# barbararoessle/e2e_multi_view_matching

Hardware: AMD Instinct MI355X
Metric: image-pairs/sec @1024 kpts + pose AUC@5/10/20deg vs reference (higher is better)
Workload: dtype f16x2 (fp32 operands carried as 2 fp16 planes hi + 2^-11 lo', 22 significant bits, 3 fp16-MFMA products, fp32 accumulate; same 1e-4 / bit-exact-index parity bar); 1 GPU; configs[1]: tuple_size=2 (1 pair per tuple), 1024 keypoints, 256-dim f32 descriptors, GNN 9x1 = 18 layers, 100 Sinkhorn iters, batch 32 tuples/GPU = 32 pairs/GPU, w8pt pose per pair; pairs_per_gpu=32, global_pairs=32, weights=random init (timed), identity-like for the AUC leg, parallelism=tuple-sharded x1

## Files before the change

### e2e_multi_view_matching_amd/build.py

```python
import hashlib
import os
import subprocess
import sys

HERE = os.path.dirname(os.path.abspath(__file__))
CSRC = os.path.join(HERE, "csrc")
LIB = os.path.join(HERE, "libe2emv.so")
SOURCES = ["ctx.hip", "weights.hip", "gemm.hip", "attention.hip", "gemm3.hip", "gemm_x3.hip", "gemm_h2.hip", "gemm_p2.hip", "gemm_p2c.hip", "attention_p2.hip", "attention_p2w.hip", "p2_tools.hip", "attention3.hip", "split3_api.hip", "sinkhorn.hip", "sinkhorn_stream.hip", "sinkhorn_resident.hip", "sinkhorn_regs.hip", "sinkhorn_regs2.hip", "pose.hip", "ba2view.hip", "gtmatch.hip",
           "mvinit.hip", "mvinit_device.hip", "mvba.hip", "mvba_backward.hip", "mvtracks.hip", "mvransac.hip", "ransac.hip", "superpoint.hip", "forward.hip", "train.hip", "comm.hip"]
REGISTER_WINDOW = ("sinkhorn_regs.hip", ("sinkhorn_resident128", "sinkhorn_resident2k"), 56)
REGISTER_WINDOW_W = ("sinkhorn_regs2.hip", ("sinkhorn_resident128w",), 64)
FLAGS = ["--offload-arch=gfx950", "-O3", "-std=c++17", "-fPIC", "-fvisibility=hidden", "-fvisibility-inlines-hidden", "-ffp-contract=fast", "-Wno-unused-result"]


def _stamp():
    h = hashlib.sha256()
    for f in sorted(f for f in os.listdir(CSRC) if f.endswith((".hip", ".h")) and os.path.isfile(os.path.join(CSRC, f))) + ["../../include/e2emv.h"]:
        with open(os.path.join(CSRC, f), "rb") as fh:
            h.update(fh.read())
    h.update(" ".join(FLAGS).encode())
    return h.hexdigest()


def build_library(force=False, verbose=False):
    hipcc = os.environ.get("HIPCC", "/opt/rocm/bin/hipcc")
    stamp_file = os.path.join(HERE, "csrc", ".build_stamp")
    stamp = _stamp()
    if not force and os.path.exists(LIB) and os.path.exists(stamp_file) and open(stamp_file).read() == stamp:
        return LIB
    _build(hipcc, os.path.join(HERE, "build"), LIB, verbose)
    with open(stamp_file, "w") as fh:
        fh.write(stamp)
    return LIB


def _check_window(asm_file, kernel, window, accumulation):
    import re
    txt = open(asm_file).read()
    n = 0
    for m in re.finditer(r"^(_Z\w*%s\w*):" % kernel, txt, re.M):
        end = txt.index(".end_amdhsa_kernel", m.end())
        dstart = txt.rfind(".amdhsa_kernel " + m.group(1), m.end(), end)
        if dstart < 0:
            raise RuntimeError(f"{m.group(1)}: no .amdhsa_kernel header in front of .end_amdhsa_kernel")
        body, desc = txt[m.end():dstart], txt[dstart:end]
        total = 512 if accumulation else 256
        if not re.search(r"\.amdhsa_next_free_vgpr\s+%d\b" % total, desc) or not re.search(r"\.amdhsa_accum_offset\s+256\b", desc):
            raise RuntimeError(f"{m.group(1)}: the wave is not allocated " + ("256 + 256 registers" if accumulation else "256 vector registers and no accumulation registers"))
        if not accumulation and not re.search(r"\.amdhsa_private_segment_fixed_size\s+0\b", desc):
            raise RuntimeError(f"{m.group(1)}: the kernel uses scratch memory")
        files = "va" if accumulation else "v"
        inasm = False
        for line in body.split("\n"):
            code = line.split(";")[0]
            if not accumulation:
                if re.search(r"\bscratch_\w+", code):
                    raise RuntimeError(f"{m.group(1)}: the kernel uses scratch memory: {line.strip()}")
                if re.search(r"\ba(\d+|\[\d+:\d+\])(?![\w.])", code) or "accvgpr" in code:
                    raise RuntimeError(f"{m.group(1)}: an accumulation register: {line.strip()}")
            if "#ASMSTART" in line:
                inasm = True
            elif "#ASMEND" in line:
                inasm = False
            elif not inasm:
                regs = [int(x) for x in re.findall(r"\b[%s](\d+)\b" % files, code)] + [int(x) for x in re.findall(r"\b[%s]\[\d+:(\d+)\]" % files, code)]
                if regs and max(regs) >= window:
                    raise RuntimeError(f"{m.group(1)}: compiler-generated code touches a register outside its window: {line.strip()}")
        n += 1
    if n == 0:
        raise RuntimeError(f"{kernel}: not found in {asm_file}")
    return n


def check_register_window(asm_file, kernel, window):
    return _check_window(asm_file, kernel, window, True)


def check_register_window_vgpr(asm_file, kernel, window):
    return _check_window(asm_file, kernel, window, False)


def _build(hipcc, objdir, lib, verbose):
    os.makedirs(objdir, exist_ok=True)
    if any("tgsplit" in f for f in FLAGS):
        raise RuntimeError("libe2emv is built for CU mode: -mtgsplit breaks the in-workgroup hand-off of gemm_p2c.hip")
    procs = []
    kept = (REGISTER_WINDOW[0], REGISTER_WINDOW_W[0])
    for src in SOURCES:
        obj = os.path.join(objdir, src.replace(".hip", ".o"))
        cmd = [hipcc] + FLAGS + ["-c", os.path.join(CSRC, src), "-o", obj]
        cwd = None
        if src in kept:
            stem = src.replace(".hip", "")
            cwd = os.path.join(objdir, stem + "_temps")
            os.makedirs(cwd, exist_ok=True)
            cmd.insert(1, "-save-temps=obj")
            cmd[-1] = os.path.join(cwd, stem + ".o")
        procs.append((src, obj, subprocess.Popen(cmd, stdout=subprocess.PIPE, stderr=subprocess.STDOUT, text=True, cwd=cwd)))
    objs = []
    for src, obj, p in procs:
        out, _ = p.communicate()
        if p.returncode != 0:
            raise RuntimeError(f"hipcc failed on {src}:\n{out}")
        if verbose and out.strip():
            print(out)
        objs.append(obj)
    import shutil
    for (src, kernels, window), check in ((REGISTER_WINDOW, check_register_window), (REGISTER_WINDOW_W, check_register_window_vgpr)):
        stem = src.replace(".hip", "")
        temps = os.path.join(objdir, stem + "_temps")
        shutil.copyfile(os.path.join(temps, stem + ".o"), os.path.join(objdir, stem + ".o"))
        asm_file = os.path.join(objdir, stem + ".s")
        shutil.copyfile(os.path.join(temps, stem + "-hip-amdgcn-amd-amdhsa-gfx950.s"), asm_file)
        for kernel in kernels:
            check(asm_file, kernel, window)
    vs = os.path.join(objdir, "e2emv.map")
    with open(vs, "w") as fh:
        fh.write("{ global: e2emv_*; local: *; };\n")
    cmd = [hipcc, "--offload-arch=gfx950", "-shared", "-fPIC", "-o", lib] + objs + ["-Wl,-rpath,/opt/rocm/lib", "-Wl,--version-script=" + vs]
    r = subprocess.run(cmd, stdout=subprocess.PIPE, stderr=subprocess.STDOUT, text=True)
    if r.returncode != 0:
        raise RuntimeError(f"link failed:\n{r.stdout}")
    return lib


if __name__ == "__main__":
    print(build_library(force="--force" in sys.argv, verbose=True))
```

### e2e_multi_view_matching_amd/csrc/attention_p2w.hip

```cpp
#include <algorithm>
#include <type_traits>

#include "attention_p2.h"

namespace e2emv {

typedef __attribute__((ext_vector_type(16))) float aw_f32x16;

constexpr int AW_QT = 256;
constexpr int AW_TILEB = 64 * 256;
constexpr int AW_REGB = 2 * AW_TILEB;
constexpr int AW_PART_F = 68;
constexpr float AW_SINV = 1.f / P2_QS, AW_PLOG = 7.f, AW_LIMIT = 60000.f;

__device__ __forceinline__ void aw_wait_q(p2_f16x8 (&q)[2][2][4]) {
    asm volatile("s_waitcnt vmcnt(16)"
                 : "+a"(q[0][0][0]), "+a"(q[0][0][1]), "+a"(q[0][0][2]), "+a"(q[0][0][3]), "+a"(q[0][1][0]), "+a"(q[0][1][1]), "+a"(q[0][1][2]), "+a"(q[0][1][3]),
                   "+a"(q[1][0][0]), "+a"(q[1][0][1]), "+a"(q[1][0][2]), "+a"(q[1][0][3]), "+a"(q[1][1][0]), "+a"(q[1][1][1]), "+a"(q[1][1][2]), "+a"(q[1][1][3])
                 :: "memory");
}

template <int I, int N, class F>
__device__ __forceinline__ void aw_for(F&& f) {
    if constexpr (I < N) {
        f(std::integral_constant<int, I>{});
        aw_for<I + 1, N>(f);
    }
}

__device__ __forceinline__ unsigned aw_cvt_pk(float v0, float v1) {
    const p2_f32x2 vv = {v0, v1};
    return __builtin_bit_cast(unsigned, __builtin_convertvector(vv, p2_f16x2));
}
__device__ __forceinline__ float aw_fma(float a, float b, float c) {
    float d;
    asm volatile("v_fma_f32 %0, %1, %2, %3" : "=v"(d) : "v"(a), "v"(b), "v"(c));
    return d;
}
__device__ __forceinline__ float aw_exp2(float a) {
    float d;
    asm volatile("v_exp_f32 %0, %1" : "=v"(d) : "v"(a));
    return d;
}
__device__ __forceinline__ void aw_acc(float& sum, float a) { asm volatile("v_add_f32 %0, %0, %1" : "+v"(sum) : "v"(a)); }
__device__ __forceinline__ unsigned aw_cvt_pk_v(float v0, float v1) {
    unsigned d;
    asm volatile("v_cvt_pk_f16_f32 %0, %1, %2" : "=v"(d) : "v"(v0), "v"(v1));
    return d;
}
__device__ __forceinline__ unsigned aw_mixlo(unsigned hi, float v0) {
    unsigned lo;
    asm volatile("v_fma_mixlo_f16 %0, %1, -1.0, %2 op_sel_hi:[1,0,0]" : "=v"(lo) : "v"(hi), "v"(v0));
    return lo;
}
__device__ __forceinline__ unsigned aw_mixhi(unsigned lo, unsigned hi, float v1) {
    asm volatile("v_fma_mixhi_f16 %0, %1, -1.0, %2 op_sel:[1,0,0] op_sel_hi:[1,0,0]" : "+v"(lo) : "v"(hi), "v"(v1));
    return lo;
}
__device__ __forceinline__ unsigned aw_lo(unsigned hi, float v0, float v1) {
    unsigned lo;
    asm("v_fma_mixlo_f16 %0, %1, -1.0, %2 op_sel_hi:[1,0,0]\n\tv_fma_mixhi_f16 %0, %1, -1.0, %3 op_sel:[1,0,0] op_sel_hi:[1,0,0]"
        : "=&v"(lo) : "v"(hi), "v"(v0), "v"(v1));
    return lo;
}

__device__ __forceinline__ void aw_mfma_s(aw_f32x16& c, p2_f16x8 a, p2_f16x8 b) {
    asm volatile("v_mfma_f32_32x32x16_f16 %0, %1, %2, %0" : "+v"(c) : "v"(a), "a"(b));
}
__device__ __forceinline__ void aw_mfma_s0(aw_f32x16& c, p2_f16x8 a, p2_f16x8 b) {
    asm volatile("v_mfma_f32_32x32x16_f16 %0, %1, %2, 0" : "=&v"(c) : "v"(a), "a"(b));
}
__device__ __forceinline__ void aw_mfma_o(aw_f32x16& c, p2_f16x8 a, p2_u32x4 b) {
    asm volatile("v_mfma_f32_32x32x16_f16 %0, %1, %2, %0" : "+a"(c) : "v"(a), "v"(b));
}
__device__ __forceinline__ void aw_load_q(const char* qp, p2_f16x8 (&q)[2][4]) {
    asm volatile(
        "global_load_dwordx4 %0, %8, off\n\t"
        "global_load_dwordx4 %1, %8, off offset:32\n\t"
        "global_load_dwordx4 %2, %8, off offset:128\n\t"
        "global_load_dwordx4 %3, %8, off offset:160\n\t"
        "global_load_dwordx4 %4, %8, off offset:64\n\t"
        "global_load_dwordx4 %5, %8, off offset:96\n\t"
        "global_load_dwordx4 %6, %8, off offset:192\n\t"
        "global_load_dwordx4 %7, %8, off offset:224"
        : "=&a"(q[0][0]), "=&a"(q[0][1]), "=&a"(q[0][2]), "=&a"(q[0][3]), "=&a"(q[1][0]), "=&a"(q[1][1]), "=&a"(q[1][2]), "=&a"(q[1][3])
        : "v"(qp) : "memory");
}

template <bool HAS_E, bool MULTI = true, bool PART = false>
__global__ __launch_bounds__(256, 1) void attention_p2w_kernel(AttnP2Params p) {
    extern __shared__ __attribute__((aligned(16))) char smem_aw[];

    int lin = blockIdx.x, ks = 0;
    constexpr bool part = PART;
    if constexpr (PART) {
        const int h = blockIdx.x, tpx = (8 * p.gper * p.nq - p.n_full) >> 3;
        ks = (h >> 3) / tpx;
        lin = p.n_full + 8 * ((h >> 3) % tpx) + (h & 7);
    }
    const int xcd = lin & 7, idx = lin >> 3;
    const int g = xcd * p.gper + idx / p.nq;
    if (g >= p.groups) return;
    const int qt = idx % p.nq;
    const int img = g / p.H, head = g % p.H;
    const int b = img / p.T, t = img % p.T;
    if (qt * AW_QT >= p.nv[t]) return;

    const int tid = threadIdx.x, lane = tid & 63;
    const int wave = __builtin_amdgcn_readfirstlane(tid >> 6);
    const int l31 = lane & 31, lh = lane >> 5;
    const unsigned row_b = 8u * (unsigned)p.D;

    int q_row[2];
    bool q_ok[2];
    p2_f16x8 Qf[2][2][4];
#pragma unroll
    for (int a = 0; a < 2; ++a) {
        q_row[a] = qt * AW_QT + wave * 64 + a * 32 + l31;
        q_ok[a] = q_row[a] < p.n_rows;
        const char* qp = reinterpret_cast<const char*>(p.qk) + ((int64_t)img * p.n_rows + (q_ok[a] ? q_row[a] : p.n_rows - 1)) * row_b + head * 256;
        aw_load_q(qp + lh * 16, Qf[a]);
    }
    const int q_blk = __builtin_amdgcn_readfirstlane(((int64_t)img * p.n_rows + min(qt * AW_QT + wave * 64, p.n_rows - 1)) >> 6);
    const int e_q = HAS_E ? p.EQK[q_blk * 8 + head] : 0;

    const int n_src = p.cross ? p.T - 1 : 1;
    auto src_t = [&](int si) __attribute__((always_inline)) { return !p.cross ? t : (si < t ? si : si + 1); };
    int n_tiles = 0;
    for (int si = 0; si < n_src; ++si) n_tiles += (p.nv[src_t(si)] + 63) / 64;
    int t0 = 0;
    if constexpr (PART) {
        t0 = ks * n_tiles / p.n_split;
        n_tiles = (ks + 1) * n_tiles / p.n_split - t0;
        if (n_tiles <= 0) return;
    }
    struct Cur { int si, kt, nv; unsigned kb, vb; int eb; };
    auto cur_src = [&](Cur& c) __attribute__((always_inline)) {
        const int im = b * p.T + src_t(c.si);
        c.kt = 0;
        c.nv = p.nv[src_t(c.si)];
        c.kb = (unsigned)(im * p.n_rows) * row_b;
        c.vb = (unsigned)((im * p.H + head) * 64) * (unsigned)p.n_rows * 4u;
        c.eb = (im * p.n_rows) >> 6;
    };
    auto cur_next = [&](Cur& c) __attribute__((always_inline)) {
        ++c.kt;
        if constexpr (MULTI) {
            if (c.kt * 64 >= c.nv && c.si + 1 < n_src) { ++c.si; cur_src(c); }
        }
    };
    auto cur_init = [&]() __attribute__((always_inline)) {
        Cur c;
        c.si = 0;
        cur_src(c);
        if constexpr (PART)
            for (int i = 0; i < t0; ++i) cur_next(c);
        return c;
    };

    const __amdgpu_buffer_rsrc_t rsK = __builtin_amdgcn_make_buffer_rsrc(const_cast<uint16_t*>(p.qk), 0, (int)p.qk_bytes, 0x00020000);
    const __amdgpu_buffer_rsrc_t rsV = __builtin_amdgcn_make_buffer_rsrc(const_cast<uint16_t*>(p.vt), 0, (int)p.vt_bytes, 0x00020000);
    unsigned k_vo[4], v_vo[4];
#pragma unroll
    for (int i = 0; i < 4; ++i) {
        const int row = 4 * (wave * 4 + i) + (lane >> 4);
        const unsigned c = (unsigned)((lane & 15) ^ (row & 15));
        k_vo[i] = (unsigned)row * row_b + 4u * (unsigned)p.D + (unsigned)head * 256u + c * 16u;
        v_vo[i] = (unsigned)row * (unsigned)p.n_rows * 4u + c * 16u;
    }
    auto k_so = [&](const Cur& c) __attribute__((always_inline)) { return c.kb + (unsigned)c.kt * 64u * row_b; };
    auto v_so = [&](const Cur& c) __attribute__((always_inline)) { return c.vb + (unsigned)c.kt * 256u; };
    auto k_piece = [&](int region, int i, unsigned so) __attribute__((always_inline)) { p2_glds16(rsK, smem_aw + region * AW_REGB + AW_TILEB + (wave * 4 + i) * 1024, k_vo[i], so); };
    auto v_piece = [&](int region, int i, unsigned so) __attribute__((always_inline)) { p2_glds16(rsV, smem_aw + region * AW_REGB + (wave * 4 + i) * 1024, v_vo[i], so); };
    int* const els = reinterpret_cast<int*>(smem_aw + 3 * AW_REGB);
    int ek_mine = 0, ev_mine = 0;
    if (HAS_E && tid < n_tiles) {
        int si = 0, kt = PART ? tid + t0 : tid;
        if constexpr (MULTI) {
            for (; si + 1 < n_src; ++si) {
                const int nt = (p.nv[src_t(si)] + 63) / 64;
                if (kt < nt) break;
                kt -= nt;
            }
        }
        const int blk = (((b * p.T + src_t(si)) * p.n_rows) >> 6) + kt;
        ek_mine = p.EQK[blk * 8 + 4 + head];
        if (p.EVt) ev_mine = p.EVt[blk * 4 + head];
    }
    typedef __attribute__((address_space(3))) const p2_u32x2* lds_pair_t;
    const unsigned els0 = (unsigned)(uintptr_t)(__attribute__((address_space(3))) char*)smem_aw + 3u * AW_REGB;
    auto read_e = [&](int tl) __attribute__((always_inline)) {
        return *reinterpret_cast<lds_pair_t>((uintptr_t)(els0 + 8u * (unsigned)min(tl, n_tiles - 1)));
    };

    const int kz = l31 & 15;
    const unsigned lds0 = (unsigned)(uintptr_t)(__attribute__((address_space(3))) char*)smem_aw;
    unsigned R[4][2];
#pragma unroll
    for (int s = 0; s < 4; ++s)
#pragma unroll
        for (int pl = 0; pl < 2; ++pl)
            R[s][pl] = lds0 + (unsigned)(l31 * 256 + ((((s >> 1) * 8 + pl * 4 + 2 * (s & 1) + lh) ^ kz) << 4));
    typedef __attribute__((address_space(3))) const p2_f16x8* lds_frag_t;
    auto frag = [&](int s, int pl, int imm) __attribute__((always_inline)) { return *reinterpret_cast<lds_frag_t>((uintptr_t)(R[s][pl] + (unsigned)imm)); };

    constexpr int PA[3] = {1, 0, 0};
    constexpr int PB[3] = {0, 1, 0};

    aw_f32x16 O[2][2], S[2][2];
    p2_u32x4 Pf[2][2][4];
#pragma unroll
    for (int a = 0; a < 2; ++a)
#pragma unroll
        for (int d = 0; d < 2; ++d)
#pragma unroll
            for (int r = 0; r < 16; ++r) O[a][d][r] = 0.f;
    float m_run[2] = {-1e30f, -1e30f}, l_run[2] = {0.f, 0.f};
    int e_o = 0;
    bool o_started = false;
    unsigned n_slow = 0;

    auto sm_slow = [&](auto BB, float sinv, int valid) __attribute__((always_inline)) {
        constexpr int B = decltype(BB)::value;
        asm volatile("s_nop 15" : "+v"(S[B][0]), "+v"(S[B][1]), "+a"(O[B][0]), "+a"(O[B][1]));
        if (valid < 64) {
#pragma unroll
            for (int kb = 0; kb < 2; ++kb)
#pragma unroll
                for (int r = 0; r < 16; ++r)
                    if (kb * 32 + (r & 3) + 8 * (r >> 2) + 4 * lh >= valid) S[B][kb][r] = -INFINITY;
        }
        float mx = S[B][0][0];
#pragma unroll
        for (int kb = 0; kb < 2; ++kb)
#pragma unroll
            for (int r = 0; r < 16; ++r) mx = fmaxf(mx, S[B][kb][r]);
        {
            float x = mx, y = mx;
            asm volatile("s_nop 1\n\tv_permlane32_swap_b32 %0, %1\n\ts_nop 1" : "+v"(x), "+v"(y));
            mx = fmaxf(x, y);
        }
        mx *= sinv;
        const float m_new = fmaxf(m_run[B], mx);
        const float alpha = __builtin_amdgcn_exp2f(m_run[B] - m_new);
#pragma unroll
        for (int r = 0; r < 16; ++r) { O[B][0][r] *= alpha; O[B][1][r] *= alpha; }
        const float e0 = AW_PLOG - m_new;
        float ps = 0.f;
#pragma unroll
        for (int k = 0; k < 16; ++k) {
            const int kb = k >> 3, r = 2 * (k & 7), u = 2 * kb + ((k & 7) >> 2), e = k & 3;
            const float p0 = __builtin_amdgcn_exp2f(__builtin_fmaf(S[B][kb][r], sinv, e0));
            const float p1 = __builtin_amdgcn_exp2f(__builtin_fmaf(S[B][kb][r + 1], sinv, e0));
            ps += p0 + p1;
            const P2Pair pr = p2_split_plain(p0, p1);
            Pf[B][0][u][e] = pr.hi; Pf[B][1][u][e] = pr.lo;
        }
        l_run[B] = l_run[B] * alpha + ps;
        m_run[B] = m_new;
        asm volatile("s_nop 4" : "+a"(O[B][0]), "+a"(O[B][1]));
    };

    Cur cK = cur_init(), cV = cur_init(), cS = cur_init();
    int nK = 0, nV = 0;
    auto adv_k = [&]() __attribute__((always_inline)) { if (++nK < n_tiles) cur_next(cK); };
    auto adv_v = [&]() __attribute__((always_inline)) { if (++nV < n_tiles) cur_next(cV); };
    {
        const unsigned so = k_so(cK);
#pragma unroll
        for (int i = 0; i < 4; ++i) k_piece(2, i, so);
        adv_k();
    }
#pragma unroll
    for (int r = 0; r < 2; ++r) {
        const unsigned sov = v_so(cV), sok = k_so(cK);
#pragma unroll
        for (int i = 0; i < 4; ++i) v_piece(r, i, sov);
#pragma unroll
        for (int i = 0; i < 4; ++i) k_piece(r, i, sok);
        adv_v();
        adv_k();
    }
    if (HAS_E && tid < n_tiles) { els[2 * tid] = ek_mine; els[2 * tid + 1] = ev_mine; }
    aw_wait_q(Qf);
    __syncthreads();
    p2_u32x2 e_pair = {0u, 0u};
    if constexpr (HAS_E) e_pair = read_e(0);
#pragma unroll
    for (int s = 0; s < 4; ++s)
#pragma unroll
        for (int pl = 0; pl < 2; ++pl) R[s][pl] += 2 * AW_REGB;
    {
        const float sinv = AW_SINV * p2_exp2i(e_q + __builtin_amdgcn_readfirstlane((int)e_pair[0]));
#pragma unroll
        for (int a = 0; a < 2; ++a)
#pragma unroll
            for (int s = 0; s < 4; ++s) {
                p2_f16x8 kf[2][2];
#pragma unroll
                for (int kb = 0; kb < 2; ++kb)
#pragma unroll
                    for (int pl = 0; pl < 2; ++pl) kf[kb][pl] = frag(s, pl, AW_TILEB + kb * 8192);
#pragma unroll
                for (int q = 0; q < 3; ++q)
#pragma unroll
                    for (int kb = 0; kb < 2; ++kb) {
                        if (s == 0 && q == 0) aw_mfma_s0(S[a][kb], kf[kb][PA[q]], Qf[a][PB[q]][s]);
                        else aw_mfma_s(S[a][kb], kf[kb][PA[q]], Qf[a][PB[q]][s]);
                    }
            }
        asm volatile("s_waitcnt vmcnt(8) lgkmcnt(0)\n\ts_barrier" ::: "memory");
        sm_slow(std::integral_constant<int, 0>{}, sinv, cS.nv - cS.kt * 64);
        if (cS.nv - cS.kt * 64 >= 64) {
            asm volatile("s_nop 15" : "+v"(S[1][0]), "+v"(S[1][1]));
            float mx = S[1][0][0];
#pragma unroll
            for (int kb = 0; kb < 2; ++kb)
#pragma unroll
                for (int r = 0; r < 16; ++r) mx = fmaxf(mx, S[1][kb][r]);
            float x = mx, y = mx;
            asm volatile("s_nop 1\n\tv_permlane32_swap_b32 %0, %1\n\ts_nop 1" : "+v"(x), "+v"(y));
            m_run[1] = fmaxf(x, y) * sinv;
        }
    }
#pragma unroll
    for (int s = 0; s < 4; ++s)
#pragma unroll
        for (int pl = 0; pl < 2; ++pl) R[s][pl] -= 2 * AW_REGB;
    int reg_cur = 0, seg_tile = 0;

    p2_f16x8 F[4][4];
    auto read_frag = [&](int buf, int n, int s, int kpart) __attribute__((always_inline)) {
        const int x = n & 1, pl = n < 2 ? 1 : 0;
        F[buf][2 * x + pl] = frag(s, pl, kpart * AW_TILEB + x * 8192);
    };
#pragma unroll
    for (int n = 0; n < 4; ++n) { read_frag(0, n, 0, 0); read_frag(1, n, 1, 0); }

    auto seg = [&](auto AA, auto LL) __attribute__((always_inline)) {
        constexpr int A = decltype(AA)::value, B = 1 - A;
        constexpr bool LAST = decltype(LL)::value;
        constexpr bool HAS_SM = !(LAST && A == 1);
        constexpr int NSLOT = LAST ? 24 : 48, NG = NSLOT / 6;
        constexpr int MPS = LAST ? 2 : 1;

        if (A == 0) {
            if (HAS_E && p.EVt) {
                const int e_v = __builtin_amdgcn_readfirstlane((int)e_pair[1]);
                if (__builtin_expect(o_started && e_v != e_o, 0)) {
                    const float f = e_o - e_v < -126 ? 0.f : p2_exp2i(e_o - e_v);
                    asm volatile("s_nop 15" : "+a"(O[0][0]), "+a"(O[0][1]), "+a"(O[1][0]), "+a"(O[1][1]));
#pragma unroll
                    for (int a = 0; a < 2; ++a)
#pragma unroll
                        for (int r = 0; r < 16; ++r) { O[a][0][r] *= f; O[a][1][r] *= f; }
                    asm volatile("s_nop 4" : "+a"(O[0][0]), "+a"(O[0][1]), "+a"(O[1][0]), "+a"(O[1][1]));
                }
                e_o = e_v;
                o_started = true;
            }
        }
        float sinv = AW_SINV, e0 = 0.f, ps = 0.f;
        int valid = 64;
        if (HAS_SM) {
            if (HAS_E) sinv = AW_SINV * p2_exp2i(e_q + __builtin_amdgcn_readfirstlane((int)e_pair[0]));
            if (HAS_E && A == 0 && !LAST) e_pair = read_e(seg_tile + 1);
            e0 = AW_PLOG - m_run[B];
            valid = cS.nv - cS.kt * 64;
        }
        if (HAS_SM && __builtin_expect(valid < 64, 0)) {
            asm volatile("s_nop 7" : "+v"(S[B][0]), "+v"(S[B][1]));
#pragma unroll
            for (int kb = 0; kb < 2; ++kb)
#pragma unroll
                for (int r = 0; r < 16; ++r)
                    if (kb * 32 + (r & 3) + 8 * (r >> 2) + 4 * lh >= valid) S[B][kb][r] = -INFINITY;
            asm volatile("" : "+v"(S[B][0]), "+v"(S[B][1]));
        }
        bool slow = false;
        float xa[16][2], pa[16][2], psA = 0.f, psB = 0.f, sinv_v = sinv;
        asm volatile("" : "+v"(sinv_v), "+v"(e0));
        unsigned hi_k[16], lo_k[16];
        auto micro = [&](auto MM) __attribute__((always_inline)) {
            constexpr int m = decltype(MM)::value;
            constexpr int k = m / 3, ph = m % 3;
            constexpr int kb = (k & 15) >> 3, r = 2 * (k & 7);
            if constexpr (m == 48) {
                lo_k[15] = aw_mixlo(hi_k[15], pa[15][0]);
            } else if constexpr (m == 49) {
                Pf[B][1][3][3] = aw_mixhi(lo_k[15], hi_k[15], pa[15][1]);
            } else if constexpr (ph == 0) {
                xa[k][0] = aw_fma(S[B][kb][r], sinv_v, e0);
                if constexpr (k > 0) lo_k[k - 1] = aw_mixlo(hi_k[k - 1], pa[k - 1][0]);
                xa[k][1] = aw_fma(S[B][kb][r + 1], sinv_v, e0);
            } else if constexpr (ph == 1) {
                pa[k][0] = aw_exp2(xa[k][0]);
                if constexpr (k > 0) {
                    constexpr int k1 = k - 1, u = 2 * (k1 >> 3) + ((k1 & 7) >> 2), e = k1 & 3;
                    Pf[B][1][u][e] = aw_mixhi(lo_k[k1], hi_k[k1], pa[k1][1]);
                }
                pa[k][1] = aw_exp2(xa[k][1]);
            } else {
                constexpr int u = 2 * (k >> 3) + ((k & 7) >> 2), e = k & 3;
                aw_acc(psA, pa[k][0]);
                hi_k[k] = aw_cvt_pk_v(pa[k][0], pa[k][1]);
                Pf[B][0][u][e] = hi_k[k];
                aw_acc(psB, pa[k][1]);
            }
        };

        unsigned so_v = 0, so_k = 0;
        if (A == 0 && !LAST) {
            so_v = v_so(cV);
            adv_v();
            so_k = k_so(cK);
            adv_k();
        }
        const int reg_ld = reg_cur == 0 ? 2 : reg_cur - 1;

        aw_for<0, NSLOT>([&](auto II) __attribute__((always_inline)) {
            constexpr int i = decltype(II)::value;
            constexpr int gq = i / 6, w = i % 6;
            if constexpr (i < 24) {
                constexpr int u = i / 6, q = (i % 6) / 2, db = i % 2;
                aw_mfma_o(O[A][db], F[u & 3][2 * db + PA[q]], Pf[A][PB[q]][u]);
            } else {
                constexpr int s = (i - 24) / 6, q = (i % 6) / 2, kb = i % 2;
                if constexpr (s == 0 && q == 0) aw_mfma_s0(S[A][kb], F[(4 + s) & 3][2 * kb + PA[q]], Qf[A][PB[q]][s]);
                else aw_mfma_s(S[A][kb], F[(4 + s) & 3][2 * kb + PA[q]], Qf[A][PB[q]][s]);
            }
            if constexpr (HAS_SM) {
                if constexpr (LAST) {
                    aw_for<0, MPS>([&](auto JJ) __attribute__((always_inline)) { micro(std::integral_constant<int, MPS * i + decltype(JJ)::value>{}); });
                } else if constexpr (i < 9) {
                    constexpr int m0 = i + i / 2 - (i > 0 && i % 2 == 0 ? 1 : 0);
                    micro(std::integral_constant<int, m0>{});
                    if constexpr (i >= 2 && i % 2 == 0) micro(std::integral_constant<int, m0 + 1>{});
                } else if constexpr (i < 46) {
                    micro(std::integral_constant<int, i + 4>{});
                } else if constexpr (i == 46) {
                    ps = psA;
                    aw_acc(ps, psB);
                } else if constexpr (i == 47) {
                    slow = __builtin_amdgcn_ballot_w64(!(ps < AW_LIMIT)) != 0;
                    l_run[B] += slow ? 0.f : ps;
                }
            }
            if constexpr (A == 1 && !LAST && i == 36) {
                asm volatile("s_waitcnt vmcnt(8) lgkmcnt(0)\n\ts_barrier" ::: "memory");
                const unsigned d = reg_cur == 2 ? (unsigned)(-2 * AW_REGB) : (unsigned)AW_REGB;
#pragma unroll
                for (int s = 0; s < 4; ++s)
#pragma unroll
                    for (int pl = 0; pl < 2; ++pl) R[s][pl] += d;
                reg_cur = reg_cur == 2 ? 0 : reg_cur + 1;
            }
            if constexpr (w >= 1 && w <= 4) {
                constexpr int gn = gq + 2;
                if constexpr (gn < NG) {
                    if constexpr (gn < 4) read_frag(gn & 3, w - 1, gn, 0);
                    else read_frag(gn & 3, w - 1, gn - 4, 1);
                } else if constexpr (!(LAST && A == 1)) {
                    read_frag((gn - NG) & 3, w - 1, gn - NG, 0);
                }
            }
            if constexpr (A == 0 && !LAST && i < 32 && i % 4 == 1) {
                if constexpr (i < 16) v_piece(reg_ld, i / 4, so_v);
                else k_piece(reg_ld, i / 4 - 4, so_k);
            }
            __builtin_amdgcn_sched_barrier(0);
        });

        if constexpr (HAS_SM && LAST) {
            lo_k[15] = aw_mixlo(hi_k[15], pa[15][0]);
            ps = psA + psB;
            Pf[B][1][3][3] = aw_mixhi(lo_k[15], hi_k[15], pa[15][1]);
            const bool slow = __builtin_amdgcn_ballot_w64(!(ps < AW_LIMIT)) != 0;
            l_run[B] += slow ? 0.f : ps;
            if (__builtin_expect(slow, 0)) {
                sm_slow(std::integral_constant<int, B>{}, sinv, valid);
                ++n_slow;
            }
        }
        if constexpr (HAS_SM && !LAST) {
            if (__builtin_expect(slow, 0)) {
                sm_slow(std::integral_constant<int, B>{}, sinv, valid);
                ++n_slow;
            }
        }
        if (A == 0) cur_next(cS);
    };

    for (int j = 0; j + 1 < n_tiles; ++j) {
        seg_tile = j;
        seg(std::integral_constant<int, 0>{}, std::false_type{});
        seg(std::integral_constant<int, 1>{}, std::false_type{});
    }
    seg(std::integral_constant<int, 0>{}, std::true_type{});
    seg(std::integral_constant<int, 1>{}, std::true_type{});

    asm volatile("s_waitcnt vmcnt(0)" ::: "memory");
    asm volatile("s_nop 15" : "+a"(O[0][0]), "+a"(O[0][1]), "+a"(O[1][0]), "+a"(O[1][1]));
    if constexpr (PART) {
        const int64_t rec = ((int64_t)(lin - p.n_full) * p.n_split + ks) * AW_QT;
        if (lane == 0) p.part_e[rec / 64 + wave] = e_o;
#pragma unroll
        for (int a = 0; a < 2; ++a) {
            const float l_tot = l_run[a] + __shfl_xor(l_run[a], 32);
            float* o = p.part + (rec + wave * 64 + a * 32 + l31) * AW_PART_F;
#pragma unroll
            for (int d = 0; d < 2; ++d)
#pragma unroll
                for (int gq = 0; gq < 4; ++gq)
                    *reinterpret_cast<p2_f32x4*>(o + 32 * d + 8 * gq + 4 * lh) = p2_f32x4{O[a][d][4 * gq], O[a][d][4 * gq + 1], O[a][d][4 * gq + 2], O[a][d][4 * gq + 3]};
            if (lh == 0) { o[64] = m_run[a]; o[65] = l_tot; }
        }
        if (p.stats && n_slow && lane == 0) atomicAdd(p.stats, n_slow);
        return;
    }
    if (p.EO && lane == 0 && q_ok[0]) p.EO[(((int64_t)img * p.n_rows + q_row[0]) >> 6) * 4 + head] = e_o;
#pragma unroll
    for (int a = 0; a < 2; ++a) {
        const float l_tot = l_run[a] + __shfl_xor(l_run[a], 32);
        const float inv = 1.f / (l_tot * P2_VS);
        uint16_t* op = p.out + p2_index((int64_t)img * p.n_rows + q_row[a], head * 64, p.D) + 8 * lh;
#pragma unroll
        for (int d = 0; d < 2; ++d)
#pragma unroll
            for (int kp = 0; kp < 2; ++kp) {
                const int r0 = 8 * kp, r1 = 8 * kp + 4;
                const P2Pair x0 = p2_split_scaled(O[a][d][r0] * inv, O[a][d][r0 + 1] * inv), x1 = p2_split_scaled(O[a][d][r0 + 2] * inv, O[a][d][r0 + 3] * inv);
                const P2Pair y0 = p2_split_scaled(O[a][d][r1] * inv, O[a][d][r1 + 1] * inv), y1 = p2_split_scaled(O[a][d][r1 + 2] * inv, O[a][d][r1 + 3] * inv);
                const auto h0 = __builtin_amdgcn_permlane32_swap(x0.hi, y0.hi, false, false), h1 = __builtin_amdgcn_permlane32_swap(x1.hi, y1.hi, false, false);
                const auto l0 = __builtin_amdgcn_permlane32_swap(x0.lo, y0.lo, false, false), l1 = __builtin_amdgcn_permlane32_swap(x1.lo, y1.lo, false, false);
                uint16_t* o = op + d * 64 + kp * 16;
                if (q_ok[a]) {
                    *reinterpret_cast<p2_u32x4*>(o) = p2_u32x4{h0[0], h1[0], h0[1], h1[1]};
                    *reinterpret_cast<p2_u32x4*>(o + 32) = p2_u32x4{l0[0], l1[0], l0[1], l1[1]};
                }
            }
    }
    if (p.stats && n_slow && lane == 0) atomicAdd(p.stats, n_slow);
}

__global__ __launch_bounds__(1024) void attention_p2w_combine(AttnP2Params p) {
    const int item = blockIdx.x, lin = p.n_full + item;
    const int xcd = lin & 7, idx = lin >> 3;
    const int g = xcd * p.gper + idx / p.nq;
    if (g >= p.groups) return;
    const int qt = idx % p.nq, img = g / p.H, head = g % p.H, t = img % p.T;
    if (qt * AW_QT >= p.nv[t]) return;
    const int n_src = p.cross ? p.T - 1 : 1;
    int n_tiles = 0;
    for (int si = 0; si < n_src; ++si) n_tiles += (p.nv[!p.cross ? t : (si < t ? si : si + 1)] + 63) / 64;
    const int q = threadIdx.x >> 2, dq = (threadIdx.x & 3) * 16;
    const int row = qt * AW_QT + q;
    float m = -3.0e38f;
    int e = -1000;
    for (int k = 0; k < p.n_split; ++k) {
        if ((k + 1) * n_tiles / p.n_split - k * n_tiles / p.n_split <= 0) continue;
        const int64_t rec = ((int64_t)item * p.n_split + k) * AW_QT;
        m = fmaxf(m, p.part[(rec + q) * AW_PART_F + 64]);
        e = max(e, p.part_e[rec / 64 + (q >> 6)]);
    }
    float acc[16], l = 0.f;
#pragma unroll
    for (int i = 0; i < 16; ++i) acc[i] = 0.f;
    for (int k = 0; k < p.n_split; ++k) {
        if ((k + 1) * n_tiles / p.n_split - k * n_tiles / p.n_split <= 0) continue;
        const int64_t rec = ((int64_t)item * p.n_split + k) * AW_QT;
        const float* o = p.part + (rec + q) * AW_PART_F;
        const int ek = p.part_e[rec / 64 + (q >> 6)];
        const float a = __builtin_amdgcn_exp2f(o[64] - m);
        const float ae = a * (ek - e < -126 ? 0.f : p2_exp2i(ek - e));
        l += a * o[65];
#pragma unroll
        for (int i = 0; i < 16; i += 4) {
            const p2_f32x4 v = *reinterpret_cast<const p2_f32x4*>(o + dq + i);
            acc[i] += ae * v[0]; acc[i + 1] += ae * v[1]; acc[i + 2] += ae * v[2]; acc[i + 3] += ae * v[3];
        }
    }
    if (row >= p.n_rows) return;
    if (p.EO && (threadIdx.x & 255) == 0) p.EO[(((int64_t)img * p.n_rows + row) >> 6) * 4 + head] = e;
    const float inv = 1.f / (l * P2_VS);
    uint16_t* op = p.out + p2_index((int64_t)img * p.n_rows + row, head * 64 + dq, p.D);
#pragma unroll
    for (int h = 0; h < 2; ++h) {
        p2_u32x4 hi, lo;
#pragma unroll
        for (int i = 0; i < 4; ++i) {
            const P2Pair pr = p2_split_scaled(acc[8 * h + 2 * i] * inv, acc[8 * h + 2 * i + 1] * inv);
            hi[i] = pr.hi; lo[i] = pr.lo;
        }
        *reinterpret_cast<p2_u32x4*>(op + 8 * h) = hi;
        *reinterpret_cast<p2_u32x4*>(op + 8 * h + 32) = lo;
    }
}

int launch_attention_p2w(e2emv_ctx* ctx, AttnP2Params& p, int n_valid, hipStream_t s) {
    p.nq = (n_valid + AW_QT - 1) / AW_QT;
    if (int rc = ensure_flags(ctx)) return rc;
    p.stats = ctx->d_flags + 5;
    const size_t lds = 3 * AW_REGB + 2048;
    const bool multi = p.cross && p.T > 2;
    const void* fn = p.EQK ? (multi ? reinterpret_cast<const void*>(attention_p2w_kernel<true, true>) : reinterpret_cast<const void*>(attention_p2w_kernel<true, false>))
                           : (multi ? reinterpret_cast<const void*>(attention_p2w_kernel<false, true>) : reinterpret_cast<const void*>(attention_p2w_kernel<false, false>));
    if (int rc = ensure_dynamic_lds(ctx, fn, lds)) return rc;
    void* args[] = {&p};
    const int n_items = 8 * p.gper * p.nq, cus = std::max(8, ctx->num_cus / 8 * 8);
    const int r = n_items % cus;
    int min_tiles = 1 << 30;
    for (int t = 0; t < p.T; ++t) {
        int nt = 0;
        for (int si = 0; si < p.T; ++si)
            if (p.cross ? si != t : si == t) nt += (p.nv[si] + 63) / 64;
        min_tiles = std::min(min_tiles, nt);
    }
    p.n_full = n_items;
    p.n_split = 1;
    p.part = nullptr;
    p.part_e = nullptr;
    if (ctx->attn_key_split && r > 0 && 2 * r <= cus && r % 8 == 0) {
        const int k = std::min(std::min(cus / r, 8), min_tiles);
        if (k >= 2) {
            const size_t n_rec = (size_t)r * k * AW_QT;
            const size_t need = n_rec * AW_PART_F * sizeof(float) + (n_rec / 64) * sizeof(int);
            if (need > ctx->attn_part_bytes) {
                if (ctx->d_attn_part) { E2EMV_HIP(ctx, hipStreamSynchronize(s)); (void)hipFree(ctx->d_attn_part); ctx->d_attn_part = nullptr; ctx->attn_part_bytes = 0; }
                E2EMV_HIP(ctx, hipMalloc((void**)&ctx->d_attn_part, need));
                ctx->attn_part_bytes = need;
            }
            p.n_full = n_items - r;
            p.n_split = k;
            p.part = ctx->d_attn_part;
            p.part_e = reinterpret_cast<int*>(ctx->d_attn_part + n_rec * AW_PART_F);
        }
    }
    if (p.n_full > 0) {
        E2EMV_HIP(ctx, hipLaunchKernel(fn, dim3(p.n_full), dim3(256), args, lds, s));
        E2EMV_CHECK_LAUNCH(ctx, "attention_p2w_kernel");
    }
    if (p.n_split > 1) {
        const void* fp = p.EQK ? (multi ? reinterpret_cast<const void*>(attention_p2w_kernel<true, true, true>) : reinterpret_cast<const void*>(attention_p2w_kernel<true, false, true>))
                               : (multi ? reinterpret_cast<const void*>(attention_p2w_kernel<false, true, true>) : reinterpret_cast<const void*>(attention_p2w_kernel<false, false, true>));
        if (int rc = ensure_dynamic_lds(ctx, fp, lds)) return rc;
        E2EMV_HIP(ctx, hipLaunchKernel(fp, dim3((n_items - p.n_full) * p.n_split), dim3(256), args, lds, s));
        E2EMV_CHECK_LAUNCH(ctx, "attention_p2w_kernel (parts)");
        hipLaunchKernelGGL(attention_p2w_combine, dim3(n_items - p.n_full), dim3(1024), 0, s, p);
        E2EMV_CHECK_LAUNCH(ctx, "attention_p2w_combine");
    }
    return E2EMV_OK;
}

}
```

Before: 3461 pairs/s.

## Stagger Q loads and first-tile scores in p2w attention prologue

Restructures the prologue of the p2w flash-attention kernel so the second Q half is loaded after the first K/V region issue. The first score block (a=0) and its softmax are computed while region 1 loads and Q[1] are still in flight, and the barrier moves after the second score block. Scale-exponent loads become inline-asm global loads so the compiler cannot insert its own vmcnt waits, and a build-time asm check enforces this. The intent is to hide global-load latency at the kernel start, at the cost of fragile hand-counted vmcnt accounting.

```diff
diff --git a/e2e_multi_view_matching_amd/build.py b/e2e_multi_view_matching_amd/build.py
--- a/e2e_multi_view_matching_amd/build.py
+++ b/e2e_multi_view_matching_amd/build.py
@@ -10,6 +10,7 @@
            "mvinit.hip", "mvinit_device.hip", "mvba.hip", "mvba_backward.hip", "mvtracks.hip", "mvransac.hip", "ransac.hip", "superpoint.hip", "forward.hip", "train.hip", "comm.hip"]
 REGISTER_WINDOW = ("sinkhorn_regs.hip", ("sinkhorn_resident128", "sinkhorn_resident2k"), 56)
 REGISTER_WINDOW_W = ("sinkhorn_regs2.hip", ("sinkhorn_resident128w",), 64)
+PROLOGUE_WAITS = ("attention_p2w.hip", "attention_p2w_kernel", "s_waitcnt vmcnt(8) lgkmcnt(0)")
 FLAGS = ["--offload-arch=gfx950", "-O3", "-std=c++17", "-fPIC", "-fvisibility=hidden", "-fvisibility-inlines-hidden", "-ffp-contract=fast", "-Wno-unused-result"]
 
 
@@ -80,12 +81,34 @@
     return _check_window(asm_file, kernel, window, False)
 
 
+def check_prologue_waits(asm_file, kernel, end_marker):
+    import re
+    txt = open(asm_file).read()
+    n = 0
+    for m in re.finditer(r"^(_Z\w*%s\w*):" % kernel, txt, re.M):
+        end = txt.find(end_marker, m.end())
+        if end < 0 or end > txt.index(".end_amdhsa_kernel", m.end()):
+            raise RuntimeError(f"{m.group(1)}: no '{end_marker}' in the kernel")
+        inasm = False
+        for line in txt[m.end():end].split("\n"):
+            if "#ASMSTART" in line:
+                inasm = True
+            elif "#ASMEND" in line:
+                inasm = False
+            elif not inasm and re.search(r"\bs_waitcnt\b.*\bvmcnt\b", line.split(";")[0]):
+                raise RuntimeError(f"{m.group(1)}: a vector-memory wait of the compiler's in the prologue: {line.strip()}")
+        n += 1
+    if n == 0:
+        raise RuntimeError(f"{kernel}: not found in {asm_file}")
+    return n
+
+
 def _build(hipcc, objdir, lib, verbose):
     os.makedirs(objdir, exist_ok=True)
     if any("tgsplit" in f for f in FLAGS):
         raise RuntimeError("libe2emv is built for CU mode: -mtgsplit breaks the in-workgroup hand-off of gemm_p2c.hip")
     procs = []
-    kept = (REGISTER_WINDOW[0], REGISTER_WINDOW_W[0])
+    kept = (REGISTER_WINDOW[0], REGISTER_WINDOW_W[0], PROLOGUE_WAITS[0])
     for src in SOURCES:
         obj = os.path.join(objdir, src.replace(".hip", ".o"))
         cmd = [hipcc] + FLAGS + ["-c", os.path.join(CSRC, src), "-o", obj]
@@ -106,7 +129,8 @@
             print(out)
         objs.append(obj)
     import shutil
-    for (src, kernels, window), check in ((REGISTER_WINDOW, check_register_window), (REGISTER_WINDOW_W, check_register_window_vgpr)):
+    for (src, kernels, window), check in ((REGISTER_WINDOW, check_register_window), (REGISTER_WINDOW_W, check_register_window_vgpr),
+                                          ((PROLOGUE_WAITS[0], PROLOGUE_WAITS[1:2], PROLOGUE_WAITS[2]), check_prologue_waits)):
         stem = src.replace(".hip", "")
         temps = os.path.join(objdir, stem + "_temps")
         shutil.copyfile(os.path.join(temps, stem + ".o"), os.path.join(objdir, stem + ".o"))
diff --git a/e2e_multi_view_matching_amd/csrc/attention_p2w.hip b/e2e_multi_view_matching_amd/csrc/attention_p2w.hip
--- a/e2e_multi_view_matching_amd/csrc/attention_p2w.hip
+++ b/e2e_multi_view_matching_amd/csrc/attention_p2w.hip
@@ -13,11 +13,20 @@
 constexpr int AW_PART_F = 68;
 constexpr float AW_SINV = 1.f / P2_QS, AW_PLOG = 7.f, AW_LIMIT = 60000.f;
 
-__device__ __forceinline__ void aw_wait_q(p2_f16x8 (&q)[2][2][4]) {
+__device__ __forceinline__ void aw_wait_q0(p2_f16x8 (&q)[2][4], int& ek, int& ev) {
     asm volatile("s_waitcnt vmcnt(16)"
-                 : "+a"(q[0][0][0]), "+a"(q[0][0][1]), "+a"(q[0][0][2]), "+a"(q[0][0][3]), "+a"(q[0][1][0]), "+a"(q[0][1][1]), "+a"(q[0][1][2]), "+a"(q[0][1][3]),
-                   "+a"(q[1][0][0]), "+a"(q[1][0][1]), "+a"(q[1][0][2]), "+a"(q[1][0][3]), "+a"(q[1][1][0]), "+a"(q[1][1][1]), "+a"(q[1][1][2]), "+a"(q[1][1][3])
+                 : "+a"(q[0][0]), "+a"(q[0][1]), "+a"(q[0][2]), "+a"(q[0][3]), "+a"(q[1][0]), "+a"(q[1][1]), "+a"(q[1][2]), "+a"(q[1][3]), "+v"(ek), "+v"(ev)
                  :: "memory");
+}
+__device__ __forceinline__ void aw_wait_q1(p2_f16x8 (&q)[2][4]) {
+    asm volatile("s_waitcnt vmcnt(16)"
+                 : "+a"(q[0][0]), "+a"(q[0][1]), "+a"(q[0][2]), "+a"(q[0][3]), "+a"(q[1][0]), "+a"(q[1][1]), "+a"(q[1][2]), "+a"(q[1][3])
+                 :: "memory");
+}
+__device__ __forceinline__ int aw_load_e(const int* ep) {
+    int e;
+    asm volatile("global_load_dword %0, %1, off" : "=&v"(e) : "v"(ep) : "memory");
+    return e;
 }
 
 template <int I, int N, class F>
@@ -111,18 +120,19 @@
     const int l31 = lane & 31, lh = lane >> 5;
     const unsigned row_b = 8u * (unsigned)p.D;
 
+    const int q_blk = __builtin_amdgcn_readfirstlane(((int64_t)img * p.n_rows + min(qt * AW_QT + wave * 64, p.n_rows - 1)) >> 6);
+    const int e_q = HAS_E ? p.EQK[q_blk * 8 + head] : 0;
     int q_row[2];
     bool q_ok[2];
+    const char* q_ptr[2];
     p2_f16x8 Qf[2][2][4];
 #pragma unroll
     for (int a = 0; a < 2; ++a) {
         q_row[a] = qt * AW_QT + wave * 64 + a * 32 + l31;
         q_ok[a] = q_row[a] < p.n_rows;
-        const char* qp = reinterpret_cast<const char*>(p.qk) + ((int64_t)img * p.n_rows + (q_ok[a] ? q_row[a] : p.n_rows - 1)) * row_b + head * 256;
-        aw_load_q(qp + lh * 16, Qf[a]);
-    }
-    const int q_blk = __builtin_amdgcn_readfirstlane(((int64_t)img * p.n_rows + min(qt * AW_QT + wave * 64, p.n_rows - 1)) >> 6);
-    const int e_q = HAS_E ? p.EQK[q_blk * 8 + head] : 0;
+        q_ptr[a] = reinterpret_cast<const char*>(p.qk) + ((int64_t)img * p.n_rows + (q_ok[a] ? q_row[a] : p.n_rows - 1)) * row_b + head * 256 + lh * 16;
+    }
+    aw_load_q(q_ptr[0], Qf[0]);
 
     const int n_src = p.cross ? p.T - 1 : 1;
     auto src_t = [&](int si) __attribute__((always_inline)) { return !p.cross ? t : (si < t ? si : si + 1); };
@@ -184,8 +194,8 @@
             }
         }
         const int blk = (((b * p.T + src_t(si)) * p.n_rows) >> 6) + kt;
-        ek_mine = p.EQK[blk * 8 + 4 + head];
-        if (p.EVt) ev_mine = p.EVt[blk * 4 + head];
+        ek_mine = aw_load_e(p.EQK + blk * 8 + 4 + head);
+        if (p.EVt) ev_mine = aw_load_e(p.EVt + blk * 4 + head);
     }
     typedef __attribute__((address_space(3))) const p2_u32x2* lds_pair_t;
     const unsigned els0 = (unsigned)(uintptr_t)(__attribute__((address_space(3))) char*)smem_aw + 3u * AW_REGB;
@@ -271,8 +281,8 @@
         for (int i = 0; i < 4; ++i) k_piece(2, i, so);
         adv_k();
     }
-#pragma unroll
-    for (int r = 0; r < 2; ++r) {
+    aw_load_q(q_ptr[1], Qf[1]);
+    auto region = [&](int r) __attribute__((always_inline)) {
         const unsigned sov = v_so(cV), sok = k_so(cK);
 #pragma unroll
         for (int i = 0; i < 4; ++i) v_piece(r, i, sov);
@@ -280,10 +290,11 @@
         for (int i = 0; i < 4; ++i) k_piece(r, i, sok);
         adv_v();
         adv_k();
-    }
+    };
+    region(0);
+    aw_wait_q0(Qf[0], ek_mine, ev_mine);
     if (HAS_E && tid < n_tiles) { els[2 * tid] = ek_mine; els[2 * tid + 1] = ev_mine; }
-    aw_wait_q(Qf);
-    __syncthreads();
+    asm volatile("s_waitcnt lgkmcnt(0)\n\ts_barrier" ::: "memory");
     p2_u32x2 e_pair = {0u, 0u};
     if constexpr (HAS_E) e_pair = read_e(0);
 #pragma unroll
@@ -292,8 +303,8 @@
         for (int pl = 0; pl < 2; ++pl) R[s][pl] += 2 * AW_REGB;
     {
         const float sinv = AW_SINV * p2_exp2i(e_q + __builtin_amdgcn_readfirstlane((int)e_pair[0]));
-#pragma unroll
-        for (int a = 0; a < 2; ++a)
+        auto first_scores = [&](auto AA) __attribute__((always_inline)) {
+            constexpr int a = decltype(AA)::value;
 #pragma unroll
             for (int s = 0; s < 4; ++s) {
                 p2_f16x8 kf[2][2];
@@ -309,8 +320,12 @@
                         else aw_mfma_s(S[a][kb], kf[kb][PA[q]], Qf[a][PB[q]][s]);
                     }
             }
-        asm volatile("s_waitcnt vmcnt(8) lgkmcnt(0)\n\ts_barrier" ::: "memory");
+        };
+        first_scores(std::integral_constant<int, 0>{});
+        region(1);
         sm_slow(std::integral_constant<int, 0>{}, sinv, cS.nv - cS.kt * 64);
+        aw_wait_q1(Qf[1]);
+        first_scores(std::integral_constant<int, 1>{});
         if (cS.nv - cS.kt * 64 >= 64) {
             asm volatile("s_nop 15" : "+v"(S[1][0]), "+v"(S[1][1]));
             float mx = S[1][0][0];
@@ -322,6 +337,7 @@
             asm volatile("s_nop 1\n\tv_permlane32_swap_b32 %0, %1\n\ts_nop 1" : "+v"(x), "+v"(y));
             m_run[1] = fmaxf(x, y) * sinv;
         }
+        asm volatile("s_waitcnt vmcnt(8) lgkmcnt(0)\n\ts_barrier" ::: "memory");
     }
 #pragma unroll
     for (int s = 0; s < 4; ++s)
```

After: 3480 pairs/s, median of 6. Within noise of the previous version (+0.6%).

## Hold attention K/V fragments in AGPRs with explicit ds_read and waitcnt scheduling

Applied to the files above, without the earlier changes.

Moves the shared-memory K/V fragment buffer from a 4-slot rotating VGPR array to an 8-group AGPR array. Each fragment is loaded with an inline ds_read_b128 that uses a compile-time offset, and explicit lgkmcnt waits are placed per group. The A-operand of the O and S MFMAs now comes from AGPRs. Fragments are loaded only in segment A=0 and reused by segment A=1, rather than being reloaded per segment. This relieves VGPR pressure and cuts duplicate LDS reads, at the cost of more AGPRs and hand-managed wait counts that could stall or be wrong if the counts are off.

```diff
diff --git a/e2e_multi_view_matching_amd/csrc/attention_p2w.hip b/e2e_multi_view_matching_amd/csrc/attention_p2w.hip
--- a/e2e_multi_view_matching_amd/csrc/attention_p2w.hip
+++ b/e2e_multi_view_matching_amd/csrc/attention_p2w.hip
@@ -70,8 +70,23 @@
 __device__ __forceinline__ void aw_mfma_s0(aw_f32x16& c, p2_f16x8 a, p2_f16x8 b) {
     asm volatile("v_mfma_f32_32x32x16_f16 %0, %1, %2, 0" : "=&v"(c) : "v"(a), "a"(b));
 }
-__device__ __forceinline__ void aw_mfma_o(aw_f32x16& c, p2_f16x8 a, p2_u32x4 b) {
-    asm volatile("v_mfma_f32_32x32x16_f16 %0, %1, %2, %0" : "+a"(c) : "v"(a), "v"(b));
+__device__ __forceinline__ void aw_mfma_sa(aw_f32x16& c, p2_f16x8 a, p2_f16x8 b) {
+    asm volatile("v_mfma_f32_32x32x16_f16 %0, %1, %2, %0" : "+v"(c) : "a"(a), "a"(b));
+}
+__device__ __forceinline__ void aw_mfma_sa0(aw_f32x16& c, p2_f16x8 a, p2_f16x8 b) {
+    asm volatile("v_mfma_f32_32x32x16_f16 %0, %1, %2, 0" : "=&v"(c) : "a"(a), "a"(b));
+}
+__device__ __forceinline__ void aw_mfma_oa(aw_f32x16& c, p2_f16x8 a, p2_u32x4 b) {
+    asm volatile("v_mfma_f32_32x32x16_f16 %0, %1, %2, %0" : "+a"(c) : "a"(a), "v"(b));
+}
+template <int IMM>
+__device__ __forceinline__ void aw_read_frag(p2_f16x8& d, unsigned addr) {
+    static_assert(IMM >= 0 && IMM < 65536, "ds_read offset: 16 bits");
+    asm volatile("ds_read_b128 %0, %1 offset:%2" : "=a"(d) : "v"(addr), "n"(IMM));
+}
+template <int N>
+__device__ __forceinline__ void aw_wait_frag(p2_f16x8 (&f)[4]) {
+    asm volatile("s_waitcnt lgkmcnt(%4)" : "+a"(f[0]), "+a"(f[1]), "+a"(f[2]), "+a"(f[3]) : "n"(N));
 }
 __device__ __forceinline__ void aw_load_q(const char* qp, p2_f16x8 (&q)[2][4]) {
     asm volatile(
@@ -329,13 +344,16 @@
         for (int pl = 0; pl < 2; ++pl) R[s][pl] -= 2 * AW_REGB;
     int reg_cur = 0, seg_tile = 0;
 
-    p2_f16x8 F[4][4];
-    auto read_frag = [&](int buf, int n, int s, int kpart) __attribute__((always_inline)) {
-        const int x = n & 1, pl = n < 2 ? 1 : 0;
-        F[buf][2 * x + pl] = frag(s, pl, kpart * AW_TILEB + x * 8192);
+    p2_f16x8 FA[8][4];
+    auto read_frag = [&](auto GG, auto NN, auto SS, auto KK) __attribute__((always_inline)) {
+        constexpr int G = decltype(GG)::value, N = decltype(NN)::value, S = decltype(SS)::value, KPART = decltype(KK)::value;
+        constexpr int x = N & 1, pl = N < 2 ? 1 : 0;
+        aw_read_frag<KPART * AW_TILEB + x * 8192>(FA[G][N], R[S][pl]);
     };
-#pragma unroll
-    for (int n = 0; n < 4; ++n) { read_frag(0, n, 0, 0); read_frag(1, n, 1, 0); }
+    aw_for<0, 8>([&](auto II) __attribute__((always_inline)) {
+        constexpr int g = decltype(II)::value / 4, n = decltype(II)::value % 4;
+        read_frag(std::integral_constant<int, g>{}, std::integral_constant<int, n>{}, std::integral_constant<int, g>{}, std::integral_constant<int, 0>{});
+    });
 
     auto seg = [&](auto AA, auto LL) __attribute__((always_inline)) {
         constexpr int A = decltype(AA)::value, B = 1 - A;
@@ -421,13 +439,14 @@
         aw_for<0, NSLOT>([&](auto II) __attribute__((always_inline)) {
             constexpr int i = decltype(II)::value;
             constexpr int gq = i / 6, w = i % 6;
+            if constexpr (A == 0 && w == 0) aw_wait_frag<(gq + 1 < NG ? 4 : 0)>(FA[gq]);
             if constexpr (i < 24) {
                 constexpr int u = i / 6, q = (i % 6) / 2, db = i % 2;
-                aw_mfma_o(O[A][db], F[u & 3][2 * db + PA[q]], Pf[A][PB[q]][u]);
+                aw_mfma_oa(O[A][db], FA[u][db + 2 * (1 - PA[q])], Pf[A][PB[q]][u]);
             } else {
                 constexpr int s = (i - 24) / 6, q = (i % 6) / 2, kb = i % 2;
-                if constexpr (s == 0 && q == 0) aw_mfma_s0(S[A][kb], F[(4 + s) & 3][2 * kb + PA[q]], Qf[A][PB[q]][s]);
-                else aw_mfma_s(S[A][kb], F[(4 + s) & 3][2 * kb + PA[q]], Qf[A][PB[q]][s]);
+                if constexpr (s == 0 && q == 0) aw_mfma_sa0(S[A][kb], FA[4 + s][kb + 2 * (1 - PA[q])], Qf[A][PB[q]][s]);
+                else aw_mfma_sa(S[A][kb], FA[4 + s][kb + 2 * (1 - PA[q])], Qf[A][PB[q]][s]);
             }
             if constexpr (HAS_SM) {
                 if constexpr (LAST) {
@@ -457,11 +476,12 @@
             }
             if constexpr (w >= 1 && w <= 4) {
                 constexpr int gn = gq + 2;
-                if constexpr (gn < NG) {
-                    if constexpr (gn < 4) read_frag(gn & 3, w - 1, gn, 0);
-                    else read_frag(gn & 3, w - 1, gn - 4, 1);
-                } else if constexpr (!(LAST && A == 1)) {
-                    read_frag((gn - NG) & 3, w - 1, gn - NG, 0);
+                constexpr auto N = std::integral_constant<int, w - 1>{};
+                if constexpr (A == 0 && gn < NG) {
+                    if constexpr (gn < 4) read_frag(std::integral_constant<int, gn>{}, N, std::integral_constant<int, gn>{}, std::integral_constant<int, 0>{});
+                    else read_frag(std::integral_constant<int, gn>{}, N, std::integral_constant<int, gn - 4>{}, std::integral_constant<int, 1>{});
+                } else if constexpr (A == 1 && !LAST && gn >= NG) {
+                    read_frag(std::integral_constant<int, gn - NG>{}, N, std::integral_constant<int, gn - NG>{}, std::integral_constant<int, 0>{});
                 }
             }
             if constexpr (A == 0 && !LAST && i < 32 && i % 4 == 1) {
```

New measurement: 3394 pairs/s before, 3439 pairs/s after (median of 6 runs). 1.3% higher.
